# guy3540/Acoustic_Locating_VQ-VAE

Measured on AMD Instinct MI355X. Metric: spectrograms/sec (train step), speech VQ-VAE default config, higher is better.
Workload: dtype x3mx_hb

## Files before the change

### acoustic_locating_vq-vae_amd/csrc/conv1d_f16mx.hip

```cpp
#include <stdlib.h>

#include "alvq_common.h"
#include "conv_tile.h"
#include "f16mx_common.h"
#include "nlc_host.h"

namespace alvq {

struct ConvFxArgs {
  ConvBArgs b;
  long x_plane, wp_plane, y_plane;
  int ea, eb;
  const float* out_scale;
  int* range_flag;
  unsigned long long* stamps;
  int dbg;
};

__device__ __forceinline__ void fx_join16(const u32x4& h0, const u32x4& h1, const u32x4& ql, float s_lo, float (&v)[16]) {
#pragma unroll
  for (int e = 0; e < 4; ++e) {
    float a0, a1, b0, b1;
    fx_join2(h0[e], ql[e >> 1], (e & 1) * 2, s_lo, a0, a1);
    fx_join2(h1[e], ql[2 + (e >> 1)], (e & 1) * 2, s_lo, b0, b1);
    v[2 * e] += a0;
    v[2 * e + 1] += a1;
    v[8 + 2 * e] += b0;
    v[8 + 2 * e + 1] += b1;
  }
}
__device__ __forceinline__ void fx_load_add16(const u16* ph, const unsigned char* pq, float s_lo, float (&v)[16]) {
  const u32x4 h0 = *(const u32x4*)ph, h1 = *(const u32x4*)(ph + 8);
  const u32x4 ql = *(const u32x4*)(pq + 32);
  fx_join16(h0, h1, ql, s_lo, v);
}

template <bool NOSTORE = false>
__device__ __forceinline__ void fx_store16(u16* ph, unsigned char* pq, float s_hi, float s_lo, const float (&v)[16], unsigned (&h)[8]) {
  unsigned qh[4], ql[4];
  fx_split<16>(v, s_hi, s_lo, h, qh, ql);
  if (NOSTORE) {
#pragma unroll
    for (int e = 0; e < 4; ++e) asm volatile("" ::"v"(h[e]), "v"(h[4 + e]), "v"(qh[e]), "v"(ql[e]));
    return;
  }
  *(u32x4*)ph = u32x4{h[0], h[1], h[2], h[3]};
  *(u32x4*)(ph + 8) = u32x4{h[4], h[5], h[6], h[7]};
  *(u32x4*)pq = u32x4{qh[0], qh[1], qh[2], qh[3]};
  *(u32x4*)(pq + 32) = u32x4{ql[0], ql[1], ql[2], ql[3]};
}

struct FxEpiLoads {
  u32x4 h0[4], h1[4], ql[4];
  u32x4 m0[4], m1[4];
  unsigned mb[4];
};

template <int NIN, int DBG = 0>
__device__ __forceinline__ void wave_epilogue_fx(const ConvFxArgs& ax, const f32x16 (&acc)[4][2], int m0, int r0, int lane, int wm0,
                                                 int wn0) {
  const ConvBArgs& a = ax.b;
  const int j = lane & 31, h = lane >> 5;
  const int Lp1 = a.L + 1, ndata = a.B * Lp1;
  const float s_lo = fx_pow2(ax.eb - FX_LO_SHIFT), s_hi = fx_pow2(ax.eb);
  fx_saturating_conversions();
  const int cb0 = m0 + wm0 + 16 * h;
  const long qo0 = fx_q_off(cb0);
  FxEpiLoads ld[NIN];
  unsigned watch = 0;
  bool okr[NIN], gapsr[NIN];
#pragma unroll
  for (int ni = 0; ni < NIN; ++ni) {
    int b, l;
    okr[ni] = row_valid(r0 + wn0 + ni * 32 + j, Lp1, ndata, &b, &l);
    gapsr[ni] = !__all(okr[ni]);
  }
  auto request = [&](int ni) {
    const long ro = (long)(r0 + wn0 + ni * 32 + j) * a.Mop;
    const u16* s1h = a.skip1 + ro + cb0;
    const unsigned char* s1q = (const unsigned char*)(a.skip1 + ax.y_plane) + ro * 2 + qo0 + 32;
    const u16* mkh = a.mask + ro + cb0;
    const unsigned char* mkb = a.mask_bits + ((ro + cb0) >> 3);
#pragma unroll
    for (int mi = 0; mi < 4; ++mi) {
      if (m0 + wm0 + mi * 32 >= a.Mop) continue;
      if (a.skip1) {
        ld[ni].h0[mi] = *(const u32x4*)(s1h + mi * 32);
        ld[ni].h1[mi] = *(const u32x4*)(s1h + mi * 32 + 8);
        ld[ni].ql[mi] = *(const u32x4*)(s1q + mi * 64);
      }
      if (a.mask_bits) {
        ld[ni].mb[mi] = *(const unsigned short*)(mkb + mi * 4);
      } else if (a.mask) {
        ld[ni].m0[mi] = *(const u32x4*)(mkh + mi * 32);
        ld[ni].m1[mi] = *(const u32x4*)(mkh + mi * 32 + 8);
      }
    }
  };
  auto tile = [&](int ni, int mi) {
    if (m0 + wm0 + mi * 32 >= a.Mop) return;
    const bool ok = okr[ni], gaps = gapsr[ni];
    const long ro = (long)(r0 + wn0 + ni * 32 + j) * a.Mop;
    const long hoff = ro + cb0 + mi * 32;
    const long qoff = ro * 2 + qo0 + mi * 64;
    float v[16];
#pragma unroll
    for (int e = 0; e < 4; ++e) {
      const u32x2 ra = __builtin_amdgcn_permlane32_swap(__float_as_uint(acc[mi][ni][e]), __float_as_uint(acc[mi][ni][8 + e]), false, false);
      const u32x2 rb = __builtin_amdgcn_permlane32_swap(__float_as_uint(acc[mi][ni][4 + e]), __float_as_uint(acc[mi][ni][12 + e]), false, false);
      v[e] = __uint_as_float(ra[0]);
      v[4 + e] = __uint_as_float(ra[1]);
      v[8 + e] = __uint_as_float(rb[0]);
      v[12 + e] = __uint_as_float(rb[1]);
    }
    if (a.bias) {
      const int cb = cb0 + mi * 32;
      if (m0 + wm0 + mi * 32 + 32 <= a.M) {
#pragma unroll
        for (int q = 0; q < 4; ++q) {
          const f32x4 bq = *(const f32x4*)(a.bias + cb + 4 * q);
#pragma unroll
          for (int e = 0; e < 4; ++e) v[4 * q + e] += bq[e];
        }
      } else {
#pragma unroll
        for (int e = 0; e < 16; ++e) v[e] += (cb + e < a.M) ? a.bias[cb + e] : 0.f;
      }
    }
    if (a.skip1) fx_join16(ld[ni].h0[mi], ld[ni].h1[mi], ld[ni].ql[mi], s_lo, v);
    if (a.skip2) fx_load_add16(a.skip2 + hoff, (const unsigned char*)(a.skip2 + ax.y_plane) + qoff, s_lo, v);
    if (a.relu & 1) {
#pragma unroll
      for (int e = 0; e < 16; ++e) asm("v_max_f32 %0, 0, %1" : "=v"(v[e]) : "v"(v[e]));
    }
    if (a.mask_bits) {
      const unsigned bt = ld[ni].mb[mi];
#pragma unroll
      for (int e = 0; e < 16; ++e) {
        unsigned m;
        asm("v_bfe_i32 %0, %1, %2, 1" : "=v"(m) : "v"(bt), "n"(e));
        v[e] = __uint_as_float(__float_as_uint(v[e]) & m);
      }
    } else if (a.mask) {
#pragma unroll
      for (int e = 0; e < 4; ++e) {
        v[2 * e] = fx_h2f_lo(ld[ni].m0[mi][e]) > 0.f ? v[2 * e] : 0.f;
        v[2 * e + 1] = fx_h2f_hi(ld[ni].m0[mi][e]) > 0.f ? v[2 * e + 1] : 0.f;
        v[8 + 2 * e] = fx_h2f_lo(ld[ni].m1[mi][e]) > 0.f ? v[8 + 2 * e] : 0.f;
        v[8 + 2 * e + 1] = fx_h2f_hi(ld[ni].m1[mi][e]) > 0.f ? v[8 + 2 * e + 1] : 0.f;
      }
    }
    if (gaps) {
#pragma unroll
      for (int e = 0; e < 16; ++e) v[e] = ok ? v[e] : 0.f;
    }
    unsigned hw[8];
    if (DBG && (ax.dbg & 512)) fx_store16<true>(a.y + hoff, (unsigned char*)(a.y + ax.y_plane) + qoff, s_hi, s_lo, v, hw);
    else fx_store16(a.y + hoff, (unsigned char*)(a.y + ax.y_plane) + qoff, s_hi, s_lo, v, hw);
#pragma unroll
    for (int e = 0; e < 8; ++e) fp16_watch(watch, hw[e]);
    if (a.bits_out) *(unsigned short*)(a.bits_out + (hoff >> 3)) = (unsigned short)fx_sign_bits_of_h(hw);
    if (a.y2) {
      fx_load_add16(a.post + hoff, (const unsigned char*)(a.post + ax.y_plane) + qoff, s_lo, v);
      if (gaps) {
#pragma unroll
        for (int e = 0; e < 16; ++e) v[e] = ok ? v[e] : 0.f;
      }
      fx_store16(a.y2 + hoff, (unsigned char*)(a.y2 + ax.y_plane) + qoff, s_hi, s_lo, v, hw);
    }
  };
  request(0);
  __builtin_amdgcn_sched_barrier(0);
  tile(0, 0);
  tile(0, 1);
  if (NIN > 1) {
    __builtin_amdgcn_sched_barrier(0);
    request(NIN - 1);
    __builtin_amdgcn_sched_barrier(0);
  }
  tile(0, 2);
  tile(0, 3);
  if (NIN > 1) {
    tile(NIN - 1, 0);
    tile(NIN - 1, 1);
    tile(NIN - 1, 2);
    tile(NIN - 1, 3);
  }
  fp16_report(watch, ax.range_flag);
}

template <int OUT, int KW, int DBG = 0, int NIN = 2, int MIN = 4>
__global__ __launch_bounds__(512, 2) void conv1d_f16mx_kernel(ConvFxArgs ax) {
  typedef ConvRings G;
  constexpr int RT = 128 * NIN;
  constexpr int MT = 64 * MIN;
  const int dbg = DBG ? ax.dbg : 0;
  const ConvBArgs& a = ax.b;
  extern __shared__ __attribute__((aligned(16))) unsigned char lds[];
  const int tid = threadIdx.x, lane = tid & 63;
  const int wave = __builtin_amdgcn_readfirstlane(tid >> 6);
  const int wm0 = (wave >> 2) * 32 * MIN, wn0 = (wave & 3) * 32 * NIN;

  const ConvTileOrigin o = conv_tile_origin<MT, RT>(a);
  const int m0 = o.m0, r0 = o.r0;
  const int Cp = a.Cp;
  const int srow = slab64_lane(lane).row;
  const unsigned lane_off = slab64_lane_off(lane, Cp);
  const long tap_w = (long)a.Mp128 * Cp * 2;
  const long row16 = (long)Cp * 32;
  const long wpl = ax.wp_plane * 2, xpl = ax.x_plane * 2;
  const char* const wb = (const char*)(a.wp + ((long)m0 + wave * 32) * Cp);
  const char* const xb = (const char*)(a.x + ((long)r0 - (KW - 1) / 2 + wave * 32) * Cp);
  const ConvRingStager<KW, MT, RT, true> st(wave, srow, lane_off, tap_w, row16, wpl, xpl, wb, xb);

  const int r32 = lane & 31, g = lane >> 5;
  int offA[2], offB[KW][2];
  offA[0] = slab64_frag32(r32, g, 0);
  offA[1] = slab64_frag32(r32, 2 + g, 0);
#pragma unroll
  for (int t = 0; t < KW; ++t) {
    offB[t][0] = slab64_frag32(r32, g, t);
    offB[t][1] = slab64_frag32(r32, 2 + g, t);
  }
  const unsigned char* const abase = lds + wm0 * 64;
  const unsigned char* const bbase = lds + G::XBASE + wn0 * 64;
  typedef int i32x4 __attribute__((ext_vector_type(4)));
  f16x8_t aH[4][2], bH[2][2];
  i32x8 aQ[4], bQ[2];
#define FX_RDH_A(WS, MI, KS) if ((MI) < MIN) aH[MI][KS] = *(const f16x8_t*)(abase + (WS) * G::WSTAGE + (MI) * 2048 + offA[KS]);
#define FX_RDH_B(XS, TAP, NI, KS) if ((NI) < NIN) bH[NI][KS] = *(const f16x8_t*)(bbase + (XS) * G::XSTAGE + (NI) * 2048 + offB[TAP][KS]);
#define FX_RDQ(DST, P, FIRST, SECOND)                                                           \
  {                                                                                             \
    const i32x4 q0_ = *(const i32x4*)((P) + (FIRST)), q1_ = *(const i32x4*)((P) + (SECOND));    \
    DST = __builtin_shufflevector(q0_, q1_, 0, 1, 2, 3, 4, 5, 6, 7);                            \
  }
#define FX_RDQ_A(WS, MI) if ((MI) < MIN) FX_RDQ(aQ[MI], abase + (WS) * G::WSTAGE + G::SLAB + (MI) * 2048, offA[0], offA[1])
#define FX_RDQ_B(XS, TAP, NI) if ((NI) < NIN) FX_RDQ(bQ[NI], bbase + (XS) * G::XSTAGE + G::XSLAB + (NI) * 2048, offB[TAP][1], offB[TAP][0])

  int sa = g ? ax.ea - FX_LO_SHIFT : ax.ea, sb = g ? ax.eb : ax.eb - FX_LO_SHIFT;
  asm volatile("" : "+v"(sa), "+v"(sb));

  f32x16 acc[4][2];
#pragma unroll
  for (int i = 0; i < 4; ++i)
#pragma unroll
    for (int jn = 0; jn < 2; ++jn)
#pragma unroll
      for (int q = 0; q < 16; ++q) acc[i][jn][q] = 0.f;
#define FX_H(MI, NI, KS) if (DBG != 2 && (NI) < NIN && (MI) < MIN) asm("v_mfma_f32_32x32x16_f16 %0, %1, %2, %0" : "+v"(acc[MI][NI]) : "v"(aH[MI][KS]), "v"(bH[NI][KS]));
#define FX_Q(MI, NI)                                                                          \
  if ((NI) < NIN && (MI) < MIN && DBG != 3)                                                                        \
    asm("v_mfma_scale_f32_32x32x64_f8f6f4 %0, %1, %2, %0, %3, %4 op_sel_hi:[0,0,0]"            \
        : "+v"(acc[MI][NI]) : "v"(aQ[MI]), "v"(bQ[NI]), "v"(sa), "v"(sb));
#define FX_SB __builtin_amdgcn_sched_barrier(0);

  const int nch = Cp / G::K;
  const int n = nch * KW;
  const bool early = wave < 4;

  unsigned long long st0 = 0, st1 = 0, st2 = 0;
  if (DBG) st0 = __builtin_amdgcn_s_memrealtime();
  st.prologue(lds, n, nch);
  if (DBG) st1 = __builtin_amdgcn_s_memrealtime();
#pragma unroll
  for (int mi = 0; mi < MIN; ++mi) { FX_RDH_A(0, mi, 0) FX_RDH_A(0, mi, 1) }
#pragma unroll
  for (int ni = 0; ni < NIN; ++ni) { FX_RDH_B(0, 0, ni, 0) FX_RDH_B(0, 0, ni, 1) }

#define FX_RD(X_) if (!(dbg & 2)) { X_ }
#define FX_DMA_E(X_) if (early && !(dbg & 1)) { X_ }
#define FX_DMA_L(X_) if (!early && !(dbg & 1)) { X_ }
#define FX_TILE(WS, XS, TAP, NWS, NXS, NTAP, TW, XC, XP)                                                                 \
  FX_H(0, 0, 0) FX_SB FX_RD(FX_RDQ_B(XS, TAP, 0)) FX_SB                                                                   \
  FX_H(0, 1, 0) FX_SB FX_RD(FX_RDQ_A(WS, 0)) FX_SB                                                                        \
  FX_H(1, 0, 0) FX_SB FX_RD(FX_RDQ_B(XS, TAP, 1)) FX_SB                                                                   \
  FX_H(1, 1, 0) FX_SB FX_RD(FX_RDQ_A(WS, 1)) FX_SB                                                                        \
  FX_H(2, 0, 0) FX_SB FX_RD(FX_RDQ_A(WS, 2)) FX_SB                                                                        \
  FX_H(2, 1, 0) FX_SB FX_RD(FX_RDQ_A(WS, 3)) FX_SB                                                                        \
  FX_H(3, 0, 0) FX_H(3, 1, 0)                                                                                            \
  FX_H(0, 0, 1) FX_H(0, 1, 1) FX_H(1, 0, 1) FX_H(1, 1, 1) FX_H(2, 0, 1) FX_H(2, 1, 1) FX_H(3, 0, 1) FX_H(3, 1, 1) FX_SB   \
  if (!(dbg & 4)) {                                                                                                      \
    asm volatile("s_waitcnt vmcnt(0) lgkmcnt(0)" ::: "memory");                                                          \
    __builtin_amdgcn_s_barrier();                                                                                        \
  }                                                                                                                      \
  FX_Q(0, 0) FX_SB FX_DMA_E(if ((TW) >= 0) st.pieceW(lds, TW, 0);) FX_RD(FX_RDH_B(NXS, NTAP, 0, 0) FX_RDH_A(NWS, 0, 0)) FX_SB     \
  FX_Q(0, 1) FX_SB FX_DMA_E(if ((TW) >= 0) st.pieceW(lds, TW, 1);) FX_RD(FX_RDH_B(NXS, NTAP, 1, 0) FX_RDH_A(NWS, 1, 0)) FX_SB     \
  FX_Q(1, 0) FX_SB FX_DMA_E(if ((TW) >= 0) st.pieceW(lds, TW, 2);) FX_RD(FX_RDH_A(NWS, 2, 0) FX_RDH_A(NWS, 3, 0)) FX_SB           \
  FX_Q(1, 1) FX_SB FX_DMA_E(if ((TW) >= 0) st.pieceW(lds, TW, 3);) FX_RD(FX_RDH_B(NXS, NTAP, 0, 1) FX_RDH_B(NXS, NTAP, 1, 1)) FX_SB \
  FX_Q(2, 0) FX_SB FX_DMA_L(if ((TW) >= 0) { st.pieceW(lds, TW, 0); st.pieceW(lds, TW, 1); }) FX_RD(FX_RDH_A(NWS, 0, 1) FX_RDH_A(NWS, 1, 1)) FX_SB \
  FX_Q(2, 1) FX_SB FX_DMA_L(if ((TW) >= 0) { st.pieceW(lds, TW, 2); st.pieceW(lds, TW, 3); }) FX_RD(FX_RDH_A(NWS, 2, 1) FX_RDH_A(NWS, 3, 1)) FX_SB \
  FX_Q(3, 0) FX_SB if (!(dbg & 1) && (XC) >= 0) { st.pieceX(lds, XC, XP, 0); st.pieceX(lds, XC, XP, 1); st.pieceX(lds, XC, XP, 2); } FX_SB       \
  FX_Q(3, 1) FX_SB if (KW == 1 && !(dbg & 1) && (XC) >= 0) { st.pieceX(lds, XC, 1, 0); st.pieceX(lds, XC, 1, 1); } FX_SB

  if (KW == 3) {
    for (int c = 0; c < nch; c += 2) {
      const int t = 3 * c;
      const int x1 = c + 1 < nch ? c + 1 : -1, x2 = c + 2 < nch ? c + 2 : -1;
      FX_TILE(0, 0, 0, 1, 0, 1, (t + 2 < n ? t + 2 : -1), x1, 0)
      FX_TILE(1, 0, 1, 0, 0, 2, (t + 3 < n ? t + 3 : -1), x1, 1)
      FX_TILE(0, 0, 2, 1, 1, 0, (t + 4 < n ? t + 4 : -1), -1, 0)
      FX_TILE(1, 1, 0, 0, 1, 1, (t + 5 < n ? t + 5 : -1), x2, 0)
      FX_TILE(0, 1, 1, 1, 1, 2, (t + 6 < n ? t + 6 : -1), x2, 1)
      FX_TILE(1, 1, 2, 0, 0, 0, (t + 7 < n ? t + 7 : -1), -1, 0)
    }
  } else {
    for (int t = 0; t < n; t += 2) {
      const int a2 = t + 2 < n ? t + 2 : -1, a3 = t + 3 < n ? t + 3 : -1;
      FX_TILE(0, 0, 0, 1, 1, 0, a2, a2, 0)
      FX_TILE(1, 1, 0, 0, 0, 0, a3, a3, 0)
    }
  }
#undef FX_TILE
#undef FX_DMA_L
#undef FX_DMA_E
#undef FX_RD
#undef FX_SB
#undef FX_Q
#undef FX_H
#undef FX_RDQ_B
#undef FX_RDQ_A
#undef FX_RDQ
#undef FX_RDH_B
#undef FX_RDH_A
  asm volatile("s_nop 15\n\ts_nop 15" ::: "memory");

  if (DBG) st2 = __builtin_amdgcn_s_memrealtime();
  if (dbg & 8) {
    if (acc[0][0][0] == 12345.678f) a.y[0] = 1;
    return;
  }
  if (OUT == 0) {
    wave_epilogue_fx<NIN, DBG>(ax, acc, m0, r0, lane, wm0, wn0);
    if (DBG && (dbg & (256 | 512))) {
      asm volatile("s_waitcnt vmcnt(0)" ::: "memory");
      __syncthreads();
      if (tid == 0) {
        unsigned long long* o = ax.stamps + (long)blockIdx.x * 4;
        o[0] = st0; o[1] = st1; o[2] = st2; o[3] = __builtin_amdgcn_s_memrealtime();
      }
    }
    return;
  }
  __syncthreads();
  conv_store_ncl<true, MT, RT>(a, lds, m0, r0, tid, ax.out_scale, [&](float* Cs, int slab) {
    if ((wn0 >> 6) != slab) return;
#pragma unroll
    for (int mi = 0; mi < MIN; ++mi)
#pragma unroll
      for (int ni = 0; ni < NIN; ++ni)
#pragma unroll
        for (int q4 = 0; q4 < 4; ++q4) {
          const int rl = (wn0 & 63) + ni * 32 + r32, ml = wm0 + mi * 32 + 8 * q4 + 4 * g;
          *(f32x4*)(Cs + rl * C_SLAB_STRIDE + ml) =
              f32x4{acc[mi][ni][4 * q4], acc[mi][ni][4 * q4 + 1], acc[mi][ni][4 * q4 + 2], acc[mi][ni][4 * q4 + 3]};
        }
  });
}

__device__ int g_fx_range_flag = 0;
__device__ int g_fx_range_sticky = 0;

int* fx_range_flag_ptr() {
  static int* cache[64] = {};
  int d = 0;
  if (hipGetDevice(&d) != hipSuccess || d < 0 || d >= 64) d = 0;
  if (!cache[d]) {
    void* p = nullptr;
    if (hipGetSymbolAddress(&p, HIP_SYMBOL(g_fx_range_flag)) == hipSuccess) cache[d] = (int*)p;
  }
  return cache[d];
}

int* fx_range_sticky_ptr() {
  static int* cache[64] = {};
  int d = 0;
  if (hipGetDevice(&d) != hipSuccess || d < 0 || d >= 64) d = 0;
  if (!cache[d]) {
    void* p = nullptr;
    if (hipGetSymbolAddress(&p, HIP_SYMBOL(g_fx_range_sticky)) == hipSuccess) cache[d] = (int*)p;
  }
  return cache[d];
}

__global__ void fx_range_flag_kernel(int* out, int reset) {
  *out = g_fx_range_flag | g_fx_range_sticky;
  if (reset) { g_fx_range_flag = 0; g_fx_range_sticky = 0; }
}

__global__ __launch_bounds__(256) void ncl_to_nlc_fx_kernel(const float* x, u16* y, long plane, int B, int C, int L, int Cp,
                                                            int rows_total, int e, const float* scale) {
  __shared__ float tile[32][33];
  fx_saturating_conversions();
  int range = 0;
  const int ct = Cp / 32;
  const int r0 = (blockIdx.x / ct) * 32, c0 = (blockIdx.x % ct) * 32;
  const int tx = threadIdx.x & 31, ty = threadIdx.x >> 5;
  const int Lp1 = L + 1, ndata = B * Lp1;
  const float sc = scale ? *scale : 1.f;
#pragma unroll
  for (int i = 0; i < 4; ++i) {
    const int c = c0 + ty + 8 * i, row = r0 + tx;
    int b, l;
    const bool ok = row_valid(row, Lp1, ndata, &b, &l) && c < C;
    const float v = ok ? x[((long)b * C + c) * L + l] * sc : 0.f;
    tile[ty + 8 * i][tx] = v;
    range |= (fabsf(v) >= 65504.f ? 1 : 0) | (v != v ? 2 : 0);
  }
  if (__any(range)) {
    for (int o = 32; o > 0; o >>= 1) range |= __shfl_xor(range, o, 64);
    if ((threadIdx.x & 63) == 0) atomicOr(&g_fx_range_flag, range);
  }
  __syncthreads();
  const int rr = threadIdx.x >> 3, cq = (threadIdx.x & 7) * 4;
  const int row = r0 + rr;
  if (row < rows_total) {
    float v[4];
#pragma unroll
    for (int k = 0; k < 4; ++k) v[k] = tile[cq + k][rr];
    unsigned h[2], qh[1], ql[1];
    fx_split<4>(v, fx_pow2(e), fx_pow2(e - FX_LO_SHIFT), h, qh, ql);
    *(u32x2*)(y + (long)row * Cp + c0 + cq) = u32x2{h[0], h[1]};
    unsigned char* q = (unsigned char*)(y + plane) + (long)row * Cp * 2 + fx_q_off(c0) + cq;
    *(unsigned*)q = qh[0];
    *(unsigned*)(q + 32) = ql[0];
  }
}

__global__ __launch_bounds__(256) void nlc_to_ncl_fx_kernel(const u16* x, long plane, float* y, int B, int C, int L, int Cp,
                                                            int rows_total, int e, const float* scale) {
  __shared__ float tile[32][33];
  const int ct = Cp / 32;
  const int r0 = (blockIdx.x / ct) * 32, c0 = (blockIdx.x % ct) * 32;
  const int tx = threadIdx.x & 31, ty = threadIdx.x >> 5;
  const int Lp1 = L + 1, ndata = B * Lp1;
  const float sc = scale ? *scale : 1.f, s_lo = fx_pow2(e - FX_LO_SHIFT);
  const int rr = threadIdx.x >> 3, cq = (threadIdx.x & 7) * 4;
  const int rowq = r0 + rr;
  if (rowq < rows_total) {
    const u32x2 h = *(const u32x2*)(x + (long)rowq * Cp + c0 + cq);
    const unsigned ql = *(const unsigned*)((const unsigned char*)(x + plane) + (long)rowq * Cp * 2 + fx_q_off(c0) + cq + 32);
    float v0, v1, v2, v3;
    fx_join2(h[0], ql, 0, s_lo, v0, v1);
    fx_join2(h[1], ql, 2, s_lo, v2, v3);
    tile[rr][cq] = v0 * sc;
    tile[rr][cq + 1] = v1 * sc;
    tile[rr][cq + 2] = v2 * sc;
    tile[rr][cq + 3] = v3 * sc;
  } else {
    tile[rr][cq] = tile[rr][cq + 1] = tile[rr][cq + 2] = tile[rr][cq + 3] = 0.f;
  }
  __syncthreads();
#pragma unroll
  for (int i = 0; i < 4; ++i) {
    const int c = c0 + ty + 8 * i, row = r0 + tx;
    int b, l;
    if (row_valid(row, Lp1, ndata, &b, &l) && c < C) y[((long)b * C + c) * L + l] = tile[tx][ty + 8 * i];
  }
}

__global__ __launch_bounds__(256) void relu_mask_fx_kernel(const u16* dy, const u16* t, u16* out, long plane, int rows, int Cp) {
  const long n16 = (long)rows * Cp / 16;
  for (long i = (long)blockIdx.x * 256 + threadIdx.x; i < n16; i += (long)gridDim.x * 256) {
    const long row = (i * 16) / Cp;
    const int c = (int)((i * 16) % Cp);
    const long ro = row * Cp;
    const u32x4 m0 = *(const u32x4*)(t + ro + c), m1 = *(const u32x4*)(t + ro + c + 8);
    u32x4 h0 = *(const u32x4*)(dy + ro + c), h1 = *(const u32x4*)(dy + ro + c + 8);
    const unsigned char* qs = (const unsigned char*)(dy + plane) + ro * 2 + fx_q_off(c);
    u32x4 qh = *(const u32x4*)qs, ql = *(const u32x4*)(qs + 32);
    unsigned keep = 0;
#pragma unroll
    for (int e = 0; e < 4; ++e) {
      keep |= (fx_h2f_lo(m0[e]) > 0.f ? 1u : 0u) << (2 * e) | (fx_h2f_hi(m0[e]) > 0.f ? 1u : 0u) << (2 * e + 1);
      keep |= (fx_h2f_lo(m1[e]) > 0.f ? 1u : 0u) << (8 + 2 * e) | (fx_h2f_hi(m1[e]) > 0.f ? 1u : 0u) << (9 + 2 * e);
    }
#pragma unroll
    for (int e = 0; e < 4; ++e) {
      const unsigned k0 = (keep >> (2 * e)) & 3u, k1 = (keep >> (8 + 2 * e)) & 3u;
      h0[e] &= ((k0 & 1u) ? 0xffffu : 0u) | ((k0 & 2u) ? 0xffff0000u : 0u);
      h1[e] &= ((k1 & 1u) ? 0xffffu : 0u) | ((k1 & 2u) ? 0xffff0000u : 0u);
      const unsigned kb = (keep >> (4 * e)) & 15u;
      const unsigned bm = ((kb & 1u) ? 0xffu : 0u) | ((kb & 2u) ? 0xff00u : 0u) | ((kb & 4u) ? 0xff0000u : 0u) | ((kb & 8u) ? 0xff000000u : 0u);
      qh[e] &= bm;
      ql[e] &= bm;
    }
    *(u32x4*)(out + ro + c) = h0;
    *(u32x4*)(out + ro + c + 8) = h1;
    unsigned char* qd = (unsigned char*)(out + plane) + ro * 2 + fx_q_off(c);
    *(u32x4*)qd = qh;
    *(u32x4*)(qd + 32) = ql;
  }
}

__global__ __launch_bounds__(256) void grad_amax_kernel(const float* x, long n, float* state) {
  float m = 0.f;
  const long n4 = n >> 2, stride = (long)gridDim.x * 256;
  long i = (long)blockIdx.x * 256 + threadIdx.x;
  for (; i + 3 * stride < n4; i += 4 * stride) {
    const f32x4 a = ((const f32x4*)x)[i], b = ((const f32x4*)x)[i + stride], c = ((const f32x4*)x)[i + 2 * stride],
                d = ((const f32x4*)x)[i + 3 * stride];
#pragma unroll
    for (int k = 0; k < 4; ++k) m = fmaxf(fmaxf(m, fmaxf(fabsf(a[k]), fabsf(b[k]))), fmaxf(fabsf(c[k]), fabsf(d[k])));
  }
  for (; i < n4; i += stride) {
    const f32x4 v = ((const f32x4*)x)[i];
    m = fmaxf(fmaxf(m, fmaxf(fabsf(v[0]), fabsf(v[1]))), fmaxf(fabsf(v[2]), fabsf(v[3])));
  }
  for (long j = (n4 << 2) + (long)blockIdx.x * 256 + threadIdx.x; j < n; j += stride) m = fmaxf(m, fabsf(x[j]));
#pragma unroll
  for (int o = 32; o > 0; o >>= 1) m = fmaxf(m, __shfl_xor(m, o, 64));
  __shared__ float wm[4];
  if ((threadIdx.x & 63) == 0) wm[threadIdx.x >> 6] = m;
  __syncthreads();
  if (threadIdx.x == 0) {
    m = fmaxf(fmaxf(wm[0], wm[1]), fmaxf(wm[2], wm[3]));
    if (m > 0.f) atomicMax((unsigned*)state + 2, __float_as_uint(m));
  }
}
__global__ void grad_scale_kernel(float* state) {
  const unsigned bits = ((unsigned*)state)[2];
  const float amax = __uint_as_float(bits);
  int e = 127;
  if (amax > 0.f && amax < 3.0e38f) {
    const int ea = (int)((bits >> 23) & 0xff);
    e = 127 + 8 - (ea - 127) - 1;
    e = e < 1 ? 1 : (e > 253 ? 253 : e);
  }
  state[0] = fx_pow2(e);
  state[1] = fx_pow2(254 - e);
  ((unsigned*)state)[2] = 0u;
}

}

using namespace alvq;

extern "C" int alvq_ncl_to_nlc_f16mx(const float* x, void* y, int B, int C, int L, const float* scale, void* stream) {
  if (int rc = check_nlc_dims("alvq_ncl_to_nlc_f16mx", x && y, B, C, L)) return rc;
  const NlcDims d(B, C, L);
  hipLaunchKernelGGL(ncl_to_nlc_fx_kernel, d.grid32(), dim3(256), 0, (hipStream_t)stream, x, (u16*)y, d.plane, B, C, L, d.Cp, d.rows,
                     FX_E_ACT, scale);
  return check_launch("alvq_ncl_to_nlc_f16mx");
}

extern "C" int alvq_nlc_to_ncl_f16mx(const void* x, float* y, int B, int C, int L, const float* scale, void* stream) {
  if (int rc = check_nlc_dims("alvq_nlc_to_ncl_f16mx", x && y, B, C, L)) return rc;
  const NlcDims d(B, C, L);
  hipLaunchKernelGGL(nlc_to_ncl_fx_kernel, d.grid32(), dim3(256), 0, (hipStream_t)stream, (const u16*)x, d.plane, y, B, C, L, d.Cp,
                     d.rows, FX_E_ACT, scale);
  return check_launch("alvq_nlc_to_ncl_f16mx");
}

extern "C" int alvq_f16mx_range_flag(int* out, int reset, void* stream) {
  ALVQ_REQUIRE(out, ALVQ_EINVAL, "alvq_f16mx_range_flag: null pointer");
  hipLaunchKernelGGL(fx_range_flag_kernel, dim3(1), dim3(1), 0, (hipStream_t)stream, out, reset);
  return check_launch("alvq_f16mx_range_flag");
}

extern "C" int alvq_relu_mask_f16mx(const void* dy, const void* t, void* out, int B, int C, int L, void* stream) {
  if (int rc = check_nlc_dims("alvq_relu_mask_f16mx", dy && t && out, B, C, L)) return rc;
  const NlcDims d(B, C, L);
  long gq = ((long)d.rows * d.Cp / 16 + 255) / 256;
  if (gq > 2048) gq = 2048;
  hipLaunchKernelGGL(relu_mask_fx_kernel, dim3((int)gq), dim3(256), 0, (hipStream_t)stream, (const u16*)dy, (const u16*)t, (u16*)out,
                     d.plane, d.rows, d.Cp);
  return check_launch("alvq_relu_mask_f16mx");
}

extern "C" int alvq_grad_scale_f32(const float* x, int64_t n, float* state, void* stream) {
  ALVQ_REQUIRE(x && state, ALVQ_EINVAL, "alvq_grad_scale_f32: null pointer");
  ALVQ_REQUIRE(n > 0, ALVQ_EINVAL, "alvq_grad_scale_f32: n <= 0");
  ALVQ_REQUIRE(((uintptr_t)x & 15) == 0, ALVQ_EINVAL, "alvq_grad_scale_f32: x must be 16-byte aligned");
  long gq = (n / 4 + 256 * 4 - 1) / (256 * 4);
  if (gq > 512) gq = 512;
  if (gq < 1) gq = 1;
  hipLaunchKernelGGL(grad_amax_kernel, dim3((int)gq), dim3(256), 0, (hipStream_t)stream, x, (long)n, state);
  hipLaunchKernelGGL(grad_scale_kernel, dim3(1), dim3(1), 0, (hipStream_t)stream, state);
  return check_launch("alvq_grad_scale_f32");
}

static constexpr int fx_slot(int OUT, int KW, int NIN, int MIN) { return (((NIN == 1) + (MIN == 2)) * 2 + OUT) * 2 + (KW == 3); }
typedef KernelTable<void (*)(ConvFxArgs), 12> FxTable;
static FxTable fx_table() {
  FxTable t;
  for_values<1, 3>([&](auto kw) {
    for_values<0, 1>([&](auto out) { for_values<2, 1>([&](auto nin) {
      t.put(fx_slot(out, kw, nin, 4), conv1d_f16mx_kernel<out, kw, 0, nin, 4>, ConvRings::LDS);
    }); });
    t.put(fx_slot(1, kw, 1, 2), conv1d_f16mx_kernel<1, kw, 0, 1, 2>, ConvRings::LDS);
  });
  return t;
}

extern "C" int alvq_conv1d_f16mx(const void* x, const void* wp, const float* bias, const void* skip1, const void* skip2,
                                 const void* mask, const void* post, void* y, void* y2, float* y_ncl, int B, int C, int M, int L,
                                 int KW, int relu, const void* mask_bits, void* relu_bits_out, const float* out_scale, void* stream) {
  if (int rc = check_conv_args("alvq_conv1d_f16mx", x, wp, skip1, skip2, mask, post, y, y2, y_ncl, B, C, M, L, KW, relu, mask_bits,
                               relu_bits_out, " (and the output scale)"))
    return rc;
  const long rows = alvq_nlc_rows(B, L);
  ConvFxArgs a{{(const u16*)x, (const u16*)wp, bias, (const u16*)skip1, (const u16*)skip2, (const u16*)mask, (const u16*)post,
                (u16*)y, (u16*)y2, y_ncl, B, L, pad_to(C, 64), M, pad_to(M, 64), pad_to(M, WP_ROWS), relu ? 1 : 0,
                (int)(rows / ConvRings::R), pad_to(M, ConvRings::M) / ConvRings::M,
                (const unsigned char*)mask_bits, (unsigned char*)relu_bits_out},
               nlc_plane_elems(B, L, C), (long)alvq_packed_weight_elems(M, C, KW), nlc_plane_elems(B, L, M),
               FX_E_W, FX_E_ACT, out_scale, fx_range_flag_ptr(), nullptr, 0};
#ifdef ALVQ_DEBUG_KERNELS
  static const int dbg_env = getenv("ALVQ_FX_DBG") ? atoi(getenv("ALVQ_FX_DBG")) : 0;
#else
  constexpr int dbg_env = 0;
#endif
  a.dbg = dbg_env;
  hipStream_t s = (hipStream_t)stream;
  static const FxTable table = fx_table();
  static DeviceOnce attr;
  if (attr.need()) {
    table.raise_lds_limit();
#ifdef ALVQ_DEBUG_KERNELS
    (void)hipFuncSetAttribute((const void*)conv1d_f16mx_kernel<0, 3, 1>, hipFuncAttributeMaxDynamicSharedMemorySize, ConvRings::LDS);
    (void)hipFuncSetAttribute((const void*)conv1d_f16mx_kernel<0, 1, 1>, hipFuncAttributeMaxDynamicSharedMemorySize, ConvRings::LDS);
    (void)hipFuncSetAttribute((const void*)conv1d_f16mx_kernel<0, 3, 2>, hipFuncAttributeMaxDynamicSharedMemorySize, ConvRings::LDS);
    (void)hipFuncSetAttribute((const void*)conv1d_f16mx_kernel<0, 3, 3>, hipFuncAttributeMaxDynamicSharedMemorySize, ConvRings::LDS);
#endif
  }
  const int forced = (int)option(OPT_FX_ROWS);
  const bool narrow = !dbg_env && y_ncl && M <= 128 && option(OPT_FX_NARROW) != 0;
  const bool half = narrow || (!dbg_env && (forced == 128 || (forced != 256 && a.b.rtiles * a.b.mtiles < 192)));
  if (half) a.b.rtiles = (int)(rows / 128);
  const dim3 grid(a.b.rtiles * a.b.mtiles), block(512);
#ifdef ALVQ_DEBUG_KERNELS
  if (dbg_env && y) {
    static unsigned long long* stamps = nullptr;
    if ((dbg_env & (256 | 512)) && !stamps) (void)hipMalloc(&stamps, 4096 * 4 * sizeof(unsigned long long));
    a.stamps = stamps;
    if (grid.x > 4096) a.dbg &= ~(256 | 512);
    if (KW == 3 && (dbg_env & 16)) hipLaunchKernelGGL((conv1d_f16mx_kernel<0, 3, 2>), grid, block, ConvRings::LDS, s, a);
    else if (KW == 3 && (dbg_env & 32)) hipLaunchKernelGGL((conv1d_f16mx_kernel<0, 3, 3>), grid, block, ConvRings::LDS, s, a);
    else if (KW == 3) hipLaunchKernelGGL((conv1d_f16mx_kernel<0, 3, 1>), grid, block, ConvRings::LDS, s, a);
    else hipLaunchKernelGGL((conv1d_f16mx_kernel<0, 1, 1>), grid, block, ConvRings::LDS, s, a);
    if (a.dbg & (256 | 512)) {
      (void)hipStreamSynchronize(s);
      static unsigned long long h[4096 * 4];
      (void)hipMemcpy(h, stamps, grid.x * 4 * sizeof(unsigned long long), hipMemcpyDeviceToHost);
      unsigned long long t0 = ~0ull, t1 = 0;
      for (unsigned i = 0; i < grid.x; ++i) { if (h[4 * i] < t0) t0 = h[4 * i]; if (h[4 * i + 3] > t1) t1 = h[4 * i + 3]; }
      double pro[2] = {0, 0}, mainl[2] = {0, 0}, epi[2] = {0, 0}, start[2] = {0, 0}; int cnt[2] = {0, 0};
      for (unsigned i = 0; i < grid.x; ++i) {
        const int rnd = (h[4 * i] - t0) * 4 > (t1 - t0) ? 1 : 0;
        pro[rnd] += h[4 * i + 1] - h[4 * i]; mainl[rnd] += h[4 * i + 2] - h[4 * i + 1]; epi[rnd] += h[4 * i + 3] - h[4 * i + 2];
        start[rnd] += h[4 * i] - t0; ++cnt[rnd];
      }
      for (int r = 0; r < 2; ++r)
        if (cnt[r])
          fprintf(stderr, "[fx stamps] KW=%d M=%d C=%d round %d: %d workgroups, start +%.1f us, staging %.2f us, main loop %.2f us, epilogue %.2f us\n",
                  KW, M, C, r, cnt[r], start[r] / cnt[r] / 100.0, pro[r] / cnt[r] / 100.0, mainl[r] / cnt[r] / 100.0, epi[r] / cnt[r] / 100.0);
      fprintf(stderr, "[fx stamps] launch span %.1f us\n", (t1 - t0) / 100.0);
    }
    return check_launch("alvq_conv1d_f16mx(dbg)");
  }
#endif
  return table.launch(fx_slot(y ? 0 : 1, KW, half ? 1 : 2, narrow ? 2 : 4), grid, block, s, "alvq_conv1d_f16mx", a);
}
```

Before: 7820.

## Specialize conv epilogue per operand set with double-buffered per-tile prefetch

Adds compile-time specialized epilogue variants for the common forward cases (relu+bits_out with optional bias, skip1, or skip1+post), which remove the runtime branches. These variants prefetch bias, skip and post operands one unit ahead into a two-slot buffer and group the stores after packing. The generic path also switches from whole-row prefetch to a per-tile rolling double buffer, which lowers register pressure. The cost is more code and kernel size, and a risk that the new load scheduling lengthens epilogue latency or changes register allocation.

```diff
diff --git a/acoustic_locating_vq-vae_amd/csrc/conv1d_f16mx.hip b/acoustic_locating_vq-vae_amd/csrc/conv1d_f16mx.hip
--- a/acoustic_locating_vq-vae_amd/csrc/conv1d_f16mx.hip
+++ b/acoustic_locating_vq-vae_amd/csrc/conv1d_f16mx.hip
@@ -35,30 +35,56 @@
   fx_join16(h0, h1, ql, s_lo, v);
 }
 
-template <bool NOSTORE = false>
-__device__ __forceinline__ void fx_store16(u16* ph, unsigned char* pq, float s_hi, float s_lo, const float (&v)[16], unsigned (&h)[8]) {
+struct FxTileOut {
+  u32x4 h0, h1, qh, ql;
+};
+
+__device__ __forceinline__ void fx_pack16(float s_hi, float s_lo, const float (&v)[16], unsigned (&hw)[8], FxTileOut& o) {
   unsigned qh[4], ql[4];
-  fx_split<16>(v, s_hi, s_lo, h, qh, ql);
-  if (NOSTORE) {
-#pragma unroll
-    for (int e = 0; e < 4; ++e) asm volatile("" ::"v"(h[e]), "v"(h[4 + e]), "v"(qh[e]), "v"(ql[e]));
-    return;
-  }
-  *(u32x4*)ph = u32x4{h[0], h[1], h[2], h[3]};
-  *(u32x4*)(ph + 8) = u32x4{h[4], h[5], h[6], h[7]};
-  *(u32x4*)pq = u32x4{qh[0], qh[1], qh[2], qh[3]};
-  *(u32x4*)(pq + 32) = u32x4{ql[0], ql[1], ql[2], ql[3]};
-}
-
+  fx_split<16>(v, s_hi, s_lo, hw, qh, ql);
+  o.h0 = u32x4{hw[0], hw[1], hw[2], hw[3]};
+  o.h1 = u32x4{hw[4], hw[5], hw[6], hw[7]};
+  o.qh = u32x4{qh[0], qh[1], qh[2], qh[3]};
+  o.ql = u32x4{ql[0], ql[1], ql[2], ql[3]};
+}
+
+template <int DBG = 0>
+__device__ __forceinline__ void fx_store_tile(u16* ph, unsigned char* pq, const FxTileOut& o, int drop = 0) {
+  if (DBG && (drop & (512 | 1024))) {
+    asm volatile("" ::"v"(o.h0), "v"(o.h1));
+  } else {
+    *(u32x4*)ph = o.h0;
+    *(u32x4*)(ph + 8) = o.h1;
+  }
+  if (DBG && (drop & (512 | 2048))) {
+    asm volatile("" ::"v"(o.qh), "v"(o.ql));
+  } else {
+    *(u32x4*)pq = o.qh;
+    *(u32x4*)(pq + 32) = o.ql;
+  }
+}
+template <int DBG = 0>
+__device__ __forceinline__ void fx_store_bits(unsigned char* pb, unsigned w, int drop = 0) {
+  if (DBG && (drop & 4096)) asm volatile("" ::"v"(w));
+  else *(unsigned short*)pb = (unsigned short)w;
+}
+
+template <int TILES>
+struct FxRowOperand {
+  u32x4 h0[TILES], h1[TILES], ql[TILES];
+};
+template <>
+struct FxRowOperand<0> {};
 struct FxEpiLoads {
-  u32x4 h0[4], h1[4], ql[4];
-  u32x4 m0[4], m1[4];
-  unsigned mb[4];
+  FxRowOperand<1> s1;
+  u32x4 m0, m1;
+  unsigned mb;
 };
 
 template <int NIN, int DBG = 0>
-__device__ __forceinline__ void wave_epilogue_fx(const ConvFxArgs& ax, const f32x16 (&acc)[4][2], int m0, int r0, int lane, int wm0,
-                                                 int wn0) {
+__device__ __forceinline__ void wave_epilogue_fx_any(const ConvFxArgs& ax, const f32x16 (&acc)[4][2], int m0, int r0, int lane,
+                                                     int wm0, int wn0) {
+  asm volatile("" : "+v"(lane));
   const ConvBArgs& a = ax.b;
   const int j = lane & 31, h = lane >> 5;
   const int Lp1 = a.L + 1, ndata = a.B * Lp1;
@@ -66,7 +92,8 @@
   fx_saturating_conversions();
   const int cb0 = m0 + wm0 + 16 * h;
   const long qo0 = fx_q_off(cb0);
-  FxEpiLoads ld[NIN];
+  const int drop = DBG ? ax.dbg : 0;
+  FxEpiLoads ld[2];
   unsigned watch = 0;
   bool okr[NIN], gapsr[NIN];
 #pragma unroll
@@ -75,31 +102,28 @@
     okr[ni] = row_valid(r0 + wn0 + ni * 32 + j, Lp1, ndata, &b, &l);
     gapsr[ni] = !__all(okr[ni]);
   }
-  auto request = [&](int ni) {
+  auto request = [&](int ni, int mi) {
+    if (m0 + wm0 + mi * 32 >= a.Mop) return;
+    FxEpiLoads& d = ld[mi & 1];
     const long ro = (long)(r0 + wn0 + ni * 32 + j) * a.Mop;
-    const u16* s1h = a.skip1 + ro + cb0;
-    const unsigned char* s1q = (const unsigned char*)(a.skip1 + ax.y_plane) + ro * 2 + qo0 + 32;
-    const u16* mkh = a.mask + ro + cb0;
-    const unsigned char* mkb = a.mask_bits + ((ro + cb0) >> 3);
-#pragma unroll
-    for (int mi = 0; mi < 4; ++mi) {
-      if (m0 + wm0 + mi * 32 >= a.Mop) continue;
-      if (a.skip1) {
-        ld[ni].h0[mi] = *(const u32x4*)(s1h + mi * 32);
-        ld[ni].h1[mi] = *(const u32x4*)(s1h + mi * 32 + 8);
-        ld[ni].ql[mi] = *(const u32x4*)(s1q + mi * 64);
-      }
-      if (a.mask_bits) {
-        ld[ni].mb[mi] = *(const unsigned short*)(mkb + mi * 4);
-      } else if (a.mask) {
-        ld[ni].m0[mi] = *(const u32x4*)(mkh + mi * 32);
-        ld[ni].m1[mi] = *(const u32x4*)(mkh + mi * 32 + 8);
-      }
+    if (a.skip1) {
+      const u16* s1h = a.skip1 + ro + cb0 + mi * 32;
+      d.s1.h0[0] = *(const u32x4*)s1h;
+      d.s1.h1[0] = *(const u32x4*)(s1h + 8);
+      d.s1.ql[0] = *(const u32x4*)((const unsigned char*)(a.skip1 + ax.y_plane) + ro * 2 + qo0 + mi * 64 + 32);
+    }
+    if (a.mask_bits) {
+      d.mb = *(const unsigned short*)(a.mask_bits + ((ro + cb0) >> 3) + mi * 4);
+    } else if (a.mask) {
+      const u16* mkh = a.mask + ro + cb0 + mi * 32;
+      d.m0 = *(const u32x4*)mkh;
+      d.m1 = *(const u32x4*)(mkh + 8);
     }
   };
   auto tile = [&](int ni, int mi) {
     if (m0 + wm0 + mi * 32 >= a.Mop) return;
     const bool ok = okr[ni], gaps = gapsr[ni];
+    const FxEpiLoads& lh = ld[mi & 1];
     const long ro = (long)(r0 + wn0 + ni * 32 + j) * a.Mop;
     const long hoff = ro + cb0 + mi * 32;
     const long qoff = ro * 2 + qo0 + mi * 64;
@@ -127,14 +151,14 @@
         for (int e = 0; e < 16; ++e) v[e] += (cb + e < a.M) ? a.bias[cb + e] : 0.f;
       }
     }
-    if (a.skip1) fx_join16(ld[ni].h0[mi], ld[ni].h1[mi], ld[ni].ql[mi], s_lo, v);
+    if (a.skip1) fx_join16(lh.s1.h0[0], lh.s1.h1[0], lh.s1.ql[0], s_lo, v);
     if (a.skip2) fx_load_add16(a.skip2 + hoff, (const unsigned char*)(a.skip2 + ax.y_plane) + qoff, s_lo, v);
     if (a.relu & 1) {
 #pragma unroll
       for (int e = 0; e < 16; ++e) asm("v_max_f32 %0, 0, %1" : "=v"(v[e]) : "v"(v[e]));
     }
     if (a.mask_bits) {
-      const unsigned bt = ld[ni].mb[mi];
+      const unsigned bt = lh.mb;
 #pragma unroll
       for (int e = 0; e < 16; ++e) {
         unsigned m;
@@ -144,10 +168,10 @@
     } else if (a.mask) {
 #pragma unroll
       for (int e = 0; e < 4; ++e) {
-        v[2 * e] = fx_h2f_lo(ld[ni].m0[mi][e]) > 0.f ? v[2 * e] : 0.f;
-        v[2 * e + 1] = fx_h2f_hi(ld[ni].m0[mi][e]) > 0.f ? v[2 * e + 1] : 0.f;
-        v[8 + 2 * e] = fx_h2f_lo(ld[ni].m1[mi][e]) > 0.f ? v[8 + 2 * e] : 0.f;
-        v[8 + 2 * e + 1] = fx_h2f_hi(ld[ni].m1[mi][e]) > 0.f ? v[8 + 2 * e + 1] : 0.f;
+        v[2 * e] = fx_h2f_lo(lh.m0[e]) > 0.f ? v[2 * e] : 0.f;
+        v[2 * e + 1] = fx_h2f_hi(lh.m0[e]) > 0.f ? v[2 * e + 1] : 0.f;
+        v[8 + 2 * e] = fx_h2f_lo(lh.m1[e]) > 0.f ? v[8 + 2 * e] : 0.f;
+        v[8 + 2 * e + 1] = fx_h2f_hi(lh.m1[e]) > 0.f ? v[8 + 2 * e + 1] : 0.f;
       }
     }
     if (gaps) {
@@ -155,38 +179,163 @@
       for (int e = 0; e < 16; ++e) v[e] = ok ? v[e] : 0.f;
     }
     unsigned hw[8];
-    if (DBG && (ax.dbg & 512)) fx_store16<true>(a.y + hoff, (unsigned char*)(a.y + ax.y_plane) + qoff, s_hi, s_lo, v, hw);
-    else fx_store16(a.y + hoff, (unsigned char*)(a.y + ax.y_plane) + qoff, s_hi, s_lo, v, hw);
+    FxTileOut o;
+    fx_pack16(s_hi, s_lo, v, hw, o);
+    fx_store_tile<DBG>(a.y + hoff, (unsigned char*)(a.y + ax.y_plane) + qoff, o, drop);
 #pragma unroll
     for (int e = 0; e < 8; ++e) fp16_watch(watch, hw[e]);
-    if (a.bits_out) *(unsigned short*)(a.bits_out + (hoff >> 3)) = (unsigned short)fx_sign_bits_of_h(hw);
+    if (a.bits_out) fx_store_bits<DBG>(a.bits_out + (hoff >> 3), fx_sign_bits_of_h(hw), drop);
     if (a.y2) {
       fx_load_add16(a.post + hoff, (const unsigned char*)(a.post + ax.y_plane) + qoff, s_lo, v);
       if (gaps) {
 #pragma unroll
         for (int e = 0; e < 16; ++e) v[e] = ok ? v[e] : 0.f;
       }
-      fx_store16(a.y2 + hoff, (unsigned char*)(a.y2 + ax.y_plane) + qoff, s_hi, s_lo, v, hw);
+      fx_pack16(s_hi, s_lo, v, hw, o);
+      fx_store_tile<DBG>(a.y2 + hoff, (unsigned char*)(a.y2 + ax.y_plane) + qoff, o, drop);
+    }
+  };
+  request(0, 0);
+#pragma unroll
+  for (int t = 0; t < 4 * NIN; ++t) {
+    __builtin_amdgcn_sched_barrier(0);
+    if (t + 1 < 4 * NIN) request((t + 1) >> 2, (t + 1) & 3);
+    __builtin_amdgcn_sched_barrier(0);
+    tile(t >> 2, t & 3);
+  }
+  fp16_report(watch, ax.range_flag);
+}
+
+template <int OPS>
+struct FxOps {
+  static constexpr bool bias = OPS == 2, skip1 = OPS == 3 || OPS == 4, post = OPS == 4;
+};
+
+template <int NIN, int OPS, int DBG = 0>
+__device__ __forceinline__ void wave_epilogue_fx_set(const ConvFxArgs& ax, const f32x16 (&acc)[4][2], int m0, int r0, int lane,
+                                                     int wm0, int wn0) {
+  typedef FxOps<OPS> O;
+  asm volatile("" : "+v"(lane));
+  const ConvBArgs& a = ax.b;
+  const int j = lane & 31, h = lane >> 5;
+  const int Lp1 = a.L + 1, ndata = a.B * Lp1;
+  const float s_lo = fx_pow2(ax.eb - FX_LO_SHIFT), s_hi = fx_pow2(ax.eb);
+  fx_saturating_conversions();
+  const int drop = DBG ? ax.dbg : 0;
+  const int cb0 = m0 + wm0 + 16 * h;
+  const long ro0 = (long)(r0 + wn0 + j) * a.Mop, rblk = (long)32 * a.Mop;
+  const long ho0 = ro0 + cb0, qo0 = ro0 * 2 + fx_q_off(cb0);
+  constexpr int U = O::post ? 1 : 2;
+  struct Unit {
+    FxRowOperand<O::skip1 ? U : 0> s1;
+    FxRowOperand<O::post ? U : 0> po;
+    f32x4 bq[O::bias ? U : 1][4];
+  } ld[2];
+  unsigned watch = 0;
+  auto request = [&](int k) {
+    Unit& d = ld[k & 1];
+#pragma unroll
+    for (int t = 0; t < U; ++t) {
+      const int ni = (U * k + t) >> 2, mi = (U * k + t) & 3;
+      if constexpr (O::bias) {
+#pragma unroll
+        for (int q = 0; q < 4; ++q) d.bq[t][q] = *(const f32x4*)(a.bias + cb0 + mi * 32 + 4 * q);
+      }
+      if constexpr (O::skip1) {
+        const u16* p = a.skip1 + ho0 + ni * rblk + mi * 32;
+        d.s1.h0[t] = *(const u32x4*)p;
+        d.s1.h1[t] = *(const u32x4*)(p + 8);
+        d.s1.ql[t] = *(const u32x4*)((const unsigned char*)(a.skip1 + ax.y_plane) + qo0 + ni * rblk * 2 + mi * 64 + 32);
+      }
+      if constexpr (O::post) {
+        const u16* p = a.post + ho0 + ni * rblk + mi * 32;
+        d.po.h0[t] = *(const u32x4*)p;
+        d.po.h1[t] = *(const u32x4*)(p + 8);
+        d.po.ql[t] = *(const u32x4*)((const unsigned char*)(a.post + ax.y_plane) + qo0 + ni * rblk * 2 + mi * 64 + 32);
+      }
     }
   };
   request(0);
   __builtin_amdgcn_sched_barrier(0);
-  tile(0, 0);
-  tile(0, 1);
-  if (NIN > 1) {
+  bool ok = true, gaps = false;
+#pragma unroll
+  for (int k = 0; k < 4 * NIN / U; ++k) {
+    const int ni = (U * k) >> 2, mi0 = (U * k) & 3;
+    const Unit& d = ld[k & 1];
+    if (mi0 == 0) {
+      int b, l;
+      ok = row_valid(r0 + wn0 + ni * 32 + j, Lp1, ndata, &b, &l);
+      gaps = !__all(ok);
+    }
+    FxTileOut out[U], out2[U];
+    unsigned bw[U];
+#pragma unroll
+    for (int t = 0; t < U; ++t) {
+      const int mi = mi0 + t;
+      float v[16];
+#pragma unroll
+      for (int e = 0; e < 4; ++e) {
+        const u32x2 ra = __builtin_amdgcn_permlane32_swap(__float_as_uint(acc[mi][ni][e]), __float_as_uint(acc[mi][ni][8 + e]), false, false);
+        const u32x2 rb = __builtin_amdgcn_permlane32_swap(__float_as_uint(acc[mi][ni][4 + e]), __float_as_uint(acc[mi][ni][12 + e]), false, false);
+        v[e] = __uint_as_float(ra[0]);
+        v[4 + e] = __uint_as_float(ra[1]);
+        v[8 + e] = __uint_as_float(rb[0]);
+        v[12 + e] = __uint_as_float(rb[1]);
+      }
+      if constexpr (O::bias) {
+#pragma unroll
+        for (int q = 0; q < 4; ++q)
+#pragma unroll
+          for (int e = 0; e < 4; ++e) v[4 * q + e] += d.bq[t][q][e];
+      }
+      if constexpr (O::skip1) fx_join16(d.s1.h0[t], d.s1.h1[t], d.s1.ql[t], s_lo, v);
+#pragma unroll
+      for (int e = 0; e < 16; ++e) asm("v_max_f32 %0, 0, %1" : "=v"(v[e]) : "v"(v[e]));
+      if (gaps) {
+#pragma unroll
+        for (int e = 0; e < 16; ++e) v[e] = ok ? v[e] : 0.f;
+      }
+      unsigned hw[8];
+      fx_pack16(s_hi, s_lo, v, hw, out[t]);
+#pragma unroll
+      for (int e = 0; e < 8; ++e) fp16_watch(watch, hw[e]);
+      bw[t] = fx_sign_bits_of_h(hw);
+      if constexpr (O::post) {
+        fx_join16(d.po.h0[t], d.po.h1[t], d.po.ql[t], s_lo, v);
+        if (gaps) {
+#pragma unroll
+          for (int e = 0; e < 16; ++e) v[e] = ok ? v[e] : 0.f;
+        }
+        fx_pack16(s_hi, s_lo, v, hw, out2[t]);
+      }
+      if (t == 0 && k + 1 < 4 * NIN / U) {
+        __builtin_amdgcn_sched_barrier(0);
+        request(k + 1);
+        __builtin_amdgcn_sched_barrier(0);
+      }
+    }
     __builtin_amdgcn_sched_barrier(0);
-    request(NIN - 1);
-    __builtin_amdgcn_sched_barrier(0);
-  }
-  tile(0, 2);
-  tile(0, 3);
-  if (NIN > 1) {
-    tile(NIN - 1, 0);
-    tile(NIN - 1, 1);
-    tile(NIN - 1, 2);
-    tile(NIN - 1, 3);
+    const long ho = ho0 + ni * rblk + mi0 * 32, qo = qo0 + ni * rblk * 2 + mi0 * 64;
+#pragma unroll
+    for (int t = 0; t < U; ++t) {
+      fx_store_tile<DBG>(a.y + ho + t * 32, (unsigned char*)(a.y + ax.y_plane) + qo + t * 64, out[t], drop);
+      fx_store_bits<DBG>(a.bits_out + ((ho + t * 32) >> 3), bw[t], drop);
+      if constexpr (O::post) fx_store_tile<DBG>(a.y2 + ho + t * 32, (unsigned char*)(a.y2 + ax.y_plane) + qo + t * 64, out2[t], drop);
+    }
   }
   fp16_report(watch, ax.range_flag);
+}
+
+template <int NIN, int DBG = 0>
+__device__ __forceinline__ void wave_epilogue_fx(const ConvFxArgs& ax, const f32x16 (&acc)[4][2], int m0, int r0, int lane, int wm0,
+                                                 int wn0) {
+  const ConvBArgs& a = ax.b;
+  const bool fwd = m0 + wm0 + 128 <= a.Mop && (a.relu & 1) && a.bits_out && !a.skip2 && !a.mask && !a.mask_bits;
+  if (fwd && !a.bias && !a.skip1 && !a.y2) wave_epilogue_fx_set<NIN, 1, DBG>(ax, acc, m0, r0, lane, wm0, wn0);
+  else if (fwd && a.bias && m0 + wm0 + 128 <= a.M && !a.skip1 && !a.y2) wave_epilogue_fx_set<NIN, 2, DBG>(ax, acc, m0, r0, lane, wm0, wn0);
+  else if (fwd && !a.bias && a.skip1 && !a.y2) wave_epilogue_fx_set<NIN, 3, DBG>(ax, acc, m0, r0, lane, wm0, wn0);
+  else if (fwd && !a.bias && a.skip1 && a.y2) wave_epilogue_fx_set<NIN, 4, DBG>(ax, acc, m0, r0, lane, wm0, wn0);
+  else wave_epilogue_fx_any<NIN, DBG>(ax, acc, m0, r0, lane, wm0, wn0);
 }
 
 template <int OUT, int KW, int DBG = 0, int NIN = 2, int MIN = 4>
```

Result: no change. 7893, median of 6 (+0.9%).
